# dangvansam/viet-asr

Hardware: AMD Instinct MI355X
Metric: real_time_factor (higher is better)
Workload: dtype f32 via 2xf16 split operands (22-bit significands, 3 f16 MFMA products per multiply, fp32 accumulate); 1 GPU; BASELINE configs[2]: quartznet15x5 greedy CTC, batch=64x10s 16kHz mono per GPU, wav in HBM -> collapsed ids; batch_per_gpu=64, parallelism=utterance-shard x1

## Files before the change

include/vasr_devtools.h:

```cpp
#ifndef VASR_DEVTOOLS_H_
#define VASR_DEVTOOLS_H_
#include "vasr.h"
#ifdef __cplusplus
extern "C" {
#endif

VASR_API int vasr_profile_bracket_overhead(vasr_stream stream, int n, double* out_us);
VASR_API int vasr_fused_tile_choice(int64_t tiles128, int compute_units);
VASR_API int vasr_fused_waves_choice(int kernel, int dual, int tile_cols);
VASR_API int vasr_bench_depthwise(const float* d_x, const float* d_w, const int32_t* d_lens, int batch, int channels,
                         int64_t frames, int kernel, float* d_y, vasr_stream stream);
VASR_API int vasr_bench_depthwise_layer(const float* d_x, const float* d_w, const int32_t* d_lens_in, const int32_t* d_lens_out,
                               int batch, int channels, int64_t frames_in, int kernel, int stride, int dilation, float* d_y,
                               uint32_t* d_amax, int amax_stride, vasr_stream stream);
VASR_API int vasr_depthwise_mfma_table_size(int kernel, int dilation);
VASR_API int vasr_pack_depthwise_taps(const float* h_w, int channels, int kernel, int dilation, uint32_t* h_table, float* h_inv);
VASR_API int vasr_bench_depthwise_mfma(const float* d_x, const uint32_t* d_taps, const float* d_tap_inv, const int32_t* d_lens,
                              int batch, int channels, int64_t frames, int kernel, int dilation, float* d_y,
                              uint32_t* d_amax, int amax_stride, vasr_stream stream);
VASR_API int vasr_pack_pointwise(const float* h_w, int cout, int cin, int m_pad, float* h_out);
VASR_API int vasr_conv_gemm_weights(const float* h_w, int cout, int cin, int kernel, float* h_out);
VASR_API int vasr_bench_pointwise(const float* d_x, const float* d_wt, const float* d_scale, const float* d_shift,
                         int batch, int cin, int cout, int64_t frames, float* d_y, vasr_stream stream);

VASR_API int vasr_bench_mfma_sustained(int gemm_mode, int workgroups, int steps, float* d_sink, double* flops, vasr_stream stream);

VASR_API int vasr_pack_pointwise_f16x2(const float* h_w, int cout, int cin, int m_pad, uint16_t* h_out, float* inv_scale);
VASR_API int vasr_bench_pointwise_f16x2(const float* d_x, const uint16_t* d_w16, float w_inv_scale, const float* d_scale,
                               const float* d_shift, int batch, int cin, int cout, int64_t frames, float* d_y,
                               uint32_t* d_amax, int amax_stride, vasr_stream stream);

VASR_API int vasr_pack_pointwise_bf16x3(const float* h_w, int cout, int cin, int m_pad, uint16_t* h_out);
VASR_API int vasr_bench_pointwise_bf16x3(const float* d_x, const uint16_t* d_w3, const float* d_scale, const float* d_shift,
                                int batch, int cin, int cout, int64_t frames, float* d_y, vasr_stream stream);

VASR_API int vasr_bench_groupnorm(const float* d_x, const int32_t* d_lens, int batch, int channels, int64_t frames,
                                  int norm_groups, int shuffle, const float* h_gamma, const float* h_beta, int relu, float* d_y,
                                  vasr_stream stream);
VASR_API int vasr_bench_ctc_head(const float* d_logits, int batch, int64_t frames, int num_classes, float* d_logp,
                                 int64_t* d_pred, vasr_stream stream);
#ifdef __cplusplus
}
#endif
#endif
```

viet-asr_amd/_lib.py:

```python
import ctypes as C
import os

import numpy as np
import torch

_HERE = os.path.dirname(os.path.abspath(__file__))
LIB_PATH = os.environ.get("VASR_LIB_PATH") or os.path.join(_HERE, "lib", "libvasr_hip.so")
DEV_LIB_PATH = os.environ.get("VASR_LIB_PATH") or os.path.join(_HERE, "lib", "libvasr_hip_dev.so")


class VasrError(RuntimeError):
    pass


class BlockDesc(C.Structure):
    _fields_ = [(n, C.c_int32) for n in
                ("filters", "repeat", "kernel", "stride", "dilation", "residual", "separable", "residual_dense")]


class FrontendDesc(C.Structure):
    _fields_ = [("sample_rate", C.c_int32), ("n_fft", C.c_int32), ("win_length", C.c_int32),
                ("hop_length", C.c_int32), ("n_mels", C.c_int32), ("preemph", C.c_float),
                ("log_guard", C.c_float), ("normalize", C.c_int32),
                ("h_window", C.POINTER(C.c_float)), ("h_filterbank", C.POINTER(C.c_float)),
# ... 66 lines not shown
    "vasr_beam_workgroups": (C.c_int, [C.c_int]),
    "vasr_beam_hash_init": (C.c_uint64, []),
    "vasr_beam_hash_step": (C.c_uint64, [C.c_uint64, C.c_uint64]),
    "vasr_last_error": (C.c_char_p, []),
    "vasr_version": (C.c_char_p, []),
    "vasr_abi_version": (C.c_int, []),
    "vasr_algorithmic_work": (C.c_int, [_P, C.c_int, C.c_int64, C.POINTER(C.c_double)]),
    "vasr_profile_begin": (C.c_int, [_P]),
    "vasr_profile_end": (C.c_int, [_P, C.POINTER(C.c_double), C.POINTER(C.c_int64), C.POINTER(C.c_double), C.POINTER(C.c_double)]),
    "vasr_padded_frames": (C.c_int64, [C.c_int64]),
}

DEV_SIGNATURES = {
    "vasr_pack_pointwise_f16x2": (C.c_int, [_P, C.c_int, C.c_int, C.c_int, _P, C.POINTER(C.c_float)]),
    "vasr_bench_pointwise_f16x2": (C.c_int, [_P, _P, C.c_float, _P, _P, C.c_int, C.c_int, C.c_int, C.c_int64, _P, _P,
                                             C.c_int, _P]),
    "vasr_depthwise_mfma_table_size": (C.c_int, [C.c_int, C.c_int]),
    "vasr_pack_depthwise_taps": (C.c_int, [_P, C.c_int, C.c_int, C.c_int, _P, _P]),
    "vasr_bench_depthwise_mfma": (C.c_int, [_P, _P, _P, _P, C.c_int, C.c_int, C.c_int64, C.c_int, C.c_int, _P, _P, C.c_int, _P]),
    "vasr_profile_bracket_overhead": (C.c_int, [_P, C.c_int, C.POINTER(C.c_double)]),
    "vasr_fused_tile_choice": (C.c_int, [C.c_int64, C.c_int]),
    "vasr_fused_waves_choice": (C.c_int, [C.c_int, C.c_int, C.c_int]),
    "vasr_pack_pointwise": (C.c_int, [_P, C.c_int, C.c_int, C.c_int, _P]),
    "vasr_conv_gemm_weights": (C.c_int, [_P, C.c_int, C.c_int, C.c_int, _P]),
    "vasr_pack_pointwise_bf16x3": (C.c_int, [_P, C.c_int, C.c_int, C.c_int, _P]),
    "vasr_bench_pointwise_bf16x3": (C.c_int, [_P, _P, _P, _P, C.c_int, C.c_int, C.c_int, C.c_int64, _P, _P]),
    "vasr_bench_mfma_sustained": (C.c_int, [C.c_int, C.c_int, C.c_int, _P, C.POINTER(C.c_double), _P]),
    "vasr_bench_depthwise": (C.c_int, [_P, _P, _P, C.c_int, C.c_int, C.c_int64, C.c_int, _P, _P]),
    "vasr_bench_depthwise_layer": (C.c_int, [_P, _P, _P, _P, C.c_int, C.c_int, C.c_int64, C.c_int, C.c_int, C.c_int, _P, _P,
                                             C.c_int, _P]),
    "vasr_bench_pointwise": (C.c_int, [_P, _P, _P, _P, C.c_int, C.c_int, C.c_int, C.c_int64, _P, _P]),
    "vasr_bench_groupnorm": (C.c_int, [_P, _P, C.c_int, C.c_int, C.c_int64, C.c_int, C.c_int, _P, _P, C.c_int, _P, _P]),
    "vasr_bench_ctc_head": (C.c_int, [_P, C.c_int, C.c_int64, C.c_int, _P, _P, _P]),
}

ABI_VERSION = 8

_lib = None
_dev = None


def _load(path, tables):
    if not os.path.exists(path):
        raise VasrError(
            f"{path} is missing: build it with `python -c 'import __graft_entry__ as g; g.build()'` "
            "(or `make -C viet-asr_amd/csrc`). There is no CPU fallback for this path.")
    l = C.CDLL(path)
    for table, required in tables:
        for name, (res, args) in table.items():
            fn = getattr(l, name, None)
            if fn is None:
                if required:
                    raise VasrError(f"{path} does not export {name}")
                continue
            fn.restype, fn.argtypes = res, args
    have = l.vasr_abi_version() if hasattr(l, "vasr_abi_version") else 0
    if have != ABI_VERSION:
        raise VasrError(f"{path} implements ABI {have}, these bindings expect {ABI_VERSION}: rebuild it (make -C viet-asr_amd/csrc)")
    return l


def lib():
    global _lib
    if _lib is None:
        _lib = _load(LIB_PATH, ((SIGNATURES, True), (DEV_SIGNATURES, False)))
    return _lib
# ... 147 lines not shown
```

viet-asr_amd/csrc/encoder_dw.hip:

```cpp
#include <cstdlib>

#include "vasr_internal.h"
#include "len_chain.h"
#include "vasr_device.h"

namespace vasr {

namespace {

constexpr int kTile = 512;

template <int K, int DIL = 1>
struct DwGeom {
  static constexpr int PAD = DIL > 1 ? (DIL * K) / 2 - 1 : K / 2;
  static constexpr int PADL = (PAD + 3) & ~3;
  static constexpr int OFF = PADL - PAD;
  static constexpr int NQ = (OFF + K + 3 + 3) / 4;
  static constexpr int WIN = 256 + 252 + 4 * NQ;
};

__device__ __forceinline__ void wave_sync() {
  __builtin_amdgcn_fence(__ATOMIC_RELEASE, "wavefront");
  __builtin_amdgcn_wave_barrier();
  __builtin_amdgcn_fence(__ATOMIC_ACQUIRE, "wavefront");
// ... 362 lines not shown
  const int t = t0 + threadIdx.x;
  int len_in = lens_in[b];
  if (len_in > frames_in) len_in = frames_in;
  const int64_t row = (int64_t)b * channels + c;
  const float* xr = x + row * ldx;
  const float* wc = w + (int64_t)c * K;
  const int span = 255 * stride + dil * (K - 1) + 1, s_base = t0 * stride - pad;
  const bool staged = span <= kSpan;
  if (staged) {
    for (int j = threadIdx.x; j < span; j += blockDim.x) {
      const int s = s_base + j;
      xs[j] = (s >= 0 && s < len_in) ? xr[s] : 0.f;
    }
    __syncthreads();
  }
  float acc = 0.f;
  if (t < ldy && t < lens_out[b]) {
    if (staged) {
      const float* xt = xs + threadIdx.x * stride;
      for (int k = 0; k < K; ++k) acc = fmaf(wc[k], xt[k * dil], acc);
    } else {
      const int s0 = t * stride - pad;
      for (int k = 0; k < K; ++k) {
        const int s = s0 + k * dil;
        if (s >= 0 && s < len_in) acc = fmaf(wc[k], xr[s], acc);
      }
    }
  }
  if (t < ldy) y[row * ldy + t] = acc;
  if (amax)
    amax_publish(amax, amax_stride, b, (c * gridDim.x + blockIdx.x) * 4 + (threadIdx.x >> 6), abs_bits(acc), threadIdx.x & 63);
}

__global__ void len_chain_kernel(const int64_t* __restrict__ seq, int batch, const LenStep* __restrict__ steps,
                                 int n_steps, int32_t* __restrict__ lens_tab, float* __restrict__ enc_len,
                                 const int64_t* __restrict__ wav_len, int hop, int frames_cap) {
  const int b = blockIdx.x * blockDim.x + threadIdx.x;
  len_chain_body(b, b < batch ? seq[b] : 0, batch, steps, n_steps, lens_tab, enc_len, wav_len, hop, frames_cap);
}

__global__ __launch_bounds__(256) void repad_kernel(const float* __restrict__ src, int64_t src_ld, int frames,
                                                    float* __restrict__ dst, int64_t dst_ld) {
  const int64_t r = blockIdx.y;
  for (int t = blockIdx.x * blockDim.x + threadIdx.x; t < dst_ld; t += gridDim.x * blockDim.x)
    dst[r * dst_ld + t] = t < frames ? src[r * src_ld + t] : 0.f;
}

template <int K>
void launch_dw_t(const float* x, int64_t ldx, const float* w, const int32_t* li, const int32_t* lo, int batch,
                 int channels, float* y, int64_t ldy, hipStream_t st, AmaxTab* amax) {
  const unsigned tiles = (unsigned)((ldy + kTile - 1) / kTile);
  unsigned* ap = amax ? amax->p : nullptr;
  const int as = amax ? amax->stride : 0;
  dim3 grid(channels / 4, batch, tiles);
  if (amax) amax->n = grid.x * 4 * tiles;
  VASR_LAUNCH((dw_conv_kernel<K, 1>), grid, dim3(256), 0, st, x, ldx, w, li, lo, channels, y, ldy, ap, as);
}

}

int depthwise_amax_slots(int channels, int64_t ldy) {
  return channels * (int)((ldy + 255) / 256) * 4;
}

static int launch_depthwise_impl(const float* x, int64_t ldx, int frames_in, const float* w, const int32_t* lens_in,
                                 const int32_t* lens_out, int batch, int channels, int kernel, int stride, int dilation,
// ... 15 lines not shown
  const bool pair = dev_switches().dw_pair;
  if (pair && aligned && stride == 1) {
    if (dilation == 2 && kernel == 87 && pad == 86)
      { launch_dw_pair<87, 2>(x, ldx, w, lens_in, lens_out, batch, channels, y, ldy, st, amax); return 0; }
    if (dilation == 1 && pad == kernel / 2) {
      switch (kernel) {
        case 33: { launch_dw_pair<33, 1>(x, ldx, w, lens_in, lens_out, batch, channels, y, ldy, st, amax); return 0; }
        case 39: { launch_dw_pair<39, 1>(x, ldx, w, lens_in, lens_out, batch, channels, y, ldy, st, amax); return 0; }
        case 51: { launch_dw_pair<51, 1>(x, ldx, w, lens_in, lens_out, batch, channels, y, ldy, st, amax); return 0; }
        case 63: { launch_dw_pair<63, 1>(x, ldx, w, lens_in, lens_out, batch, channels, y, ldy, st, amax); return 0; }
        case 75: { launch_dw_pair<75, 1>(x, ldx, w, lens_in, lens_out, batch, channels, y, ldy, st, amax); return 0; }
        default: break;
      }
    }
  }
  if (aligned && stride == 1 && dilation == 2 && kernel == 87 && pad == 86) {
    dim3 grid(channels / 4, batch, (unsigned)((ldy + kTile - 1) / kTile));
    if (amax) amax->n = grid.x * 4 * grid.z;
    VASR_LAUNCH((dw_conv_kernel<87, 1, 2>), grid, dim3(256), 0, st, x, ldx, w, lens_in, lens_out, channels,
                       y, ldy, amax ? amax->p : nullptr, amax ? amax->stride : 0);
    return 0;
  }
  const bool fast = aligned && stride == 1 && dilation == 1 && pad == kernel / 2;
  if (fast) {
    switch (kernel) {
      case 33: { launch_dw_t<33>(x, ldx, w, lens_in, lens_out, batch, channels, y, ldy, st, amax); return 0; }
      case 39: { launch_dw_t<39>(x, ldx, w, lens_in, lens_out, batch, channels, y, ldy, st, amax); return 0; }
      case 51: { launch_dw_t<51>(x, ldx, w, lens_in, lens_out, batch, channels, y, ldy, st, amax); return 0; }
      case 63: { launch_dw_t<63>(x, ldx, w, lens_in, lens_out, batch, channels, y, ldy, st, amax); return 0; }
      case 75: { launch_dw_t<75>(x, ldx, w, lens_in, lens_out, batch, channels, y, ldy, st, amax); return 0; }
      default: break;
    }
  }
  dim3 grid((unsigned)((ldy + 255) / 256), channels, batch);
  if (amax) amax->n = channels * grid.x * 4;
  VASR_LAUNCH(dw_conv_generic_kernel, grid, dim3(256), 0, st, x, ldx, frames_in, w, lens_in, lens_out,
                     channels, kernel, stride, dilation, pad, y, ldy, amax ? amax->p : nullptr, amax ? amax->stride : 0);
  return 0;
}

__global__ __launch_bounds__(256) void amax_kernel(const float* __restrict__ x, int64_t ld, int rows, int frames,
                                                   const int32_t* __restrict__ lens, unsigned* __restrict__ amax,
                                                   int amax_stride, int64_t bs) {
  const int b = blockIdx.y;
  int n = lens ? lens[b] : frames;
  n = n < frames ? n : frames;
  unsigned m = 0;
  for (int r = blockIdx.x; r < rows; r += gridDim.x) {
    const float* xr = x + (int64_t)b * bs + (int64_t)r * ld;
    for (int t = threadIdx.x; t < n; t += blockDim.x) m = max(m, abs_bits(xr[t]));
  }
  amax_publish(amax, amax_stride, b, blockIdx.x * 4 + (threadIdx.x >> 6), m, threadIdx.x & 63);
}

void launch_amax(const float* x, int64_t ld, int rows, int frames, const int32_t* lens, int batch, AmaxTab* amax,
                 hipStream_t st, int64_t batch_stride) {
  const int gx = rows < 64 ? rows : 64;
  amax->n = gx * 4;
  hipLaunchKernelGGL(amax_kernel, dim3(gx, batch), dim3(256), 0, st, x, ld, rows, frames, lens, amax->p, amax->stride,
                     batch_stride ? batch_stride : (int64_t)rows * ld);
}

void launch_len_chain(const int64_t* seq, int batch, const LenStep* d_steps, int n_steps, int32_t* lens_tab,
                      float* enc_len, hipStream_t st, const int64_t* wav_len, int hop, int frames_cap) {
  hipLaunchKernelGGL(len_chain_kernel, dim3((batch + 63) / 64), dim3(64), 0, st, seq, batch, d_steps, n_steps,
                     lens_tab, enc_len, wav_len, hop, frames_cap);
// ... 10 lines not shown
```

viet-asr_amd/csrc/vasr_api.cpp:

```cpp
#include <hip/hip_runtime.h>

#include <cmath>
#include <cstdarg>
#include <cstdio>
#include <cstdlib>
#include <cstring>
#include <map>
#include <memory>
#include <string>
#include <algorithm>
#include <vector>

#include "vasr.h"
#include "vasr_host.h"
#include "vasr_internal.h"

using namespace vasr;

namespace {
thread_local std::string g_err;
}

namespace vasr {

// ... 1053 lines not shown
      }
      int published;
      {
        ProfScope ps(h, kProfPointwise, st, 2.0 * W.cin * W.cout * (double)g_T * batch, 4.0 * W.m_pad * (double)dst_ld * batch);
        published = run_pointwise(h, a, W, st);
      }
      if (published < 0) return VASR_ERR_HIP;
      if (nrm) {
        if (run_norm(S.norm, dst, dst, (last_sub && B.has_res) ? R : nullptr, dst_ld, blk_ld, g_T, a.store_cols,
                     lens(S.pw.step + 1), enc_out ? nullptr : lens(S.pw.step + 1), act, published ? &a.amax_y : nullptr,
                     a.lens_y))
          return VASR_ERR_HIP;
      }
      if (S.se.d_w1) {
        if (run_se(S.se, dst, dst, dst_ld, g_T, a.store_cols, lens(S.pw.step + 1), enc_out ? nullptr : lens(S.pw.step + 1),
                   last_sub ? 1 : 0, 0, published ? &a.amax_y : nullptr, a.lens_y))
          return VASR_ERR_HIP;
      }
      cur = dst; cur_ld = dst_ld; cur_T = g_T;
      cur_amax = published ? a.amax_y : AmaxTab{};
    }
  }
  if (enc_amax) *enc_amax = cur_amax;
  return check_launch("encoder");
}

int run_decoder(vasr_handle* h, const float* encp, int64_t ld, int64_t T1, int batch, float* logits, float* logp,
                int64_t* pred, hipStream_t st, AmaxTab enc_amax = AmaxTab{}, const int32_t* own_frames = nullptr) {
  PwArgs a = pw_args(h, h->dec, encp, logits, ld, T1, batch);
  a.lens = own_frames;
  a.m_store = h->num_classes;
  ProfScope ps(h, kProfHead, st);
  a.amax_x = enc_amax;
  if (run_pointwise(h, a, h->dec, st) < 0) return VASR_ERR_HIP;
  launch_logsoftmax_argmax(logits, ld, (int64_t)h->num_classes * ld, batch, (int)T1, h->num_classes, logp, pred, st);
  return check_launch("decoder");
}

}

extern "C" {

const char* vasr_last_error(void) { return g_err.c_str(); }
const char* vasr_version(void) { return "vasr-hip 0.4 (gfx950)"; }
int vasr_abi_version(void) { return VASR_ABI_VERSION; }
int64_t vasr_padded_frames(int64_t frames) { return pad_frames(frames); }

int vasr_create(const vasr_model_desc* d, vasr_handle** out) {
  if (!d || !out) return fail(VASR_ERR_INVALID, "null argument");
  std::unique_ptr<vasr_handle> owner(new vasr_handle());
  vasr_handle* h = owner.get();
  if (d->frontend) {
    const vasr_frontend_desc& fe = *d->frontend;
    if (fe.n_fft != 512 || fe.n_mels != 64) {
      return fail(VASR_ERR_UNSUPPORTED, "front end supports n_fft=512, n_mels=64 (got %d, %d)", fe.n_fft, fe.n_mels);
    }
    if (fe.win_length <= 0 || fe.win_length > fe.n_fft || fe.hop_length <= 0 || fe.hop_length > 512 ||
        !fe.h_filterbank) {
      return fail(VASR_ERR_INVALID, "invalid window/hop/filterbank in front-end description");
    }
    h->has_frontend = true;
    h->fe = fe;
    h->fe_window.resize(fe.win_length);
    for (int i = 0; i < fe.win_length; ++i)
      h->fe_window[i] = fe.h_window ? fe.h_window[i]
                                    : (float)(0.5 - 0.5 * std::cos(2.0 * M_PI * i / (fe.win_length - 1)));
// ... 873 lines not shown
```

viet-asr_amd/csrc/vasr_devtools.cpp:

```cpp
#include <hip/hip_runtime.h>

#include <algorithm>
#include <cstdio>
#include <cstdlib>
#include <initializer_list>
#include <vector>

#include "vasr.h"
#include "vasr_devtools.h"
#include "vasr_host.h"
#include "vasr_internal.h"

using namespace vasr;

const vasr::DevSwitches& vasr::dev_switches() {
  static const DevSwitches sw = [] {
    DevSwitches s;
    auto num = [](const char* name, int dflt, std::initializer_list<int> allowed) {
      const char* e = getenv(name);
      if (!e) return dflt;
      const int v = atoi(e);
      for (int a : allowed) if (a == v) return v;
      fprintf(stderr, "vasr (devtools build): %s=%s is not a documented value -- refusing to guess\n", name, e);
      abort();
      return dflt;
    };
    s.pw3_tile = num("VASR_PW3_TILE", 0, {0, 1, 2, 3, 4, 5});
    s.pw_lat = num("VASR_PW_LAT", 1, {0, 1});
    s.dw_pair = num("VASR_DW_PAIR", 1, {0, 1}) != 0;
    s.dw_mfma = num("VASR_DW_MFMA", 1, {0, 1}) != 0;
    s.dw_upw = num("VASR_DW_UPW", 0, {0, 1, 2, 3, 4, 5, 6, 7, 8});
    s.fused = num("VASR_FUSED", 1, {0, 1}) != 0;
    s.fused_min_tiles = getenv("VASR_FUSED_MIN_TILES") ? atoi(getenv("VASR_FUSED_MIN_TILES")) : 0;
    s.fused_tile = num("VASR_FUSED_TILE", 0, {0, 64, 128});
    s.fused_waves = num("VASR_FUSED_WAVES", 0, {0, 8, 16});
    s.fused_residual = num("VASR_NO_FUSED_RESIDUAL", 0, {0, 1}) == 0;
    s.beam_group = num("VASR_BEAM_GROUP", -1, {-1, 0, 1, 4});
    s.no_grouped = num("VASR_NO_GROUPED", 0, {0, 1}) != 0;
    return s;
  }();
  return sw;
}

extern "C" {

int vasr_fused_tile_choice(int64_t tiles128, int compute_units) { return vasr::fused_tile_choice(tiles128, compute_units); }
int vasr_fused_waves_choice(int kernel, int dual, int tile_cols) {
  return vasr::fused_waves_choice(kernel, dual != 0, tile_cols, vasr::dev_switches().fused_waves);
}

static __global__ void dev_noop_kernel() {}

int vasr_profile_bracket_overhead(vasr_stream stream, int n, double* out_us) {
  if (n < 1 || n > 4096 || !out_us) return fail(VASR_ERR_INVALID, "bad argument");
  hipStream_t st = static_cast<hipStream_t>(stream);
  std::vector<hipEvent_t> ev(2 * (size_t)n);
  for (auto& e : ev) HIP_TRY(hipEventCreate(&e));
  for (int i = 0; i < n; ++i) {
    HIP_TRY(hipEventRecord(ev[2 * i], st));
    hipLaunchKernelGGL(dev_noop_kernel, dim3(1), dim3(64), 0, st);
    HIP_TRY(hipEventRecord(ev[2 * i + 1], st));
  }
  HIP_TRY(hipEventSynchronize(ev.back()));
  std::vector<float> t(n);
  for (int i = 0; i < n; ++i) HIP_TRY(hipEventElapsedTime(&t[i], ev[2 * i], ev[2 * i + 1]));
  for (auto& e : ev) (void)hipEventDestroy(e);
  std::sort(t.begin(), t.end());
  *out_us = 1e3 * (double)t[n / 2];
  return 0;
}

// ... 150 lines not shown
  const size_t nc = (size_t)channels, ws = (size_t)2 * batch * (channels + norm_groups);
  HIP_TRY(hipMalloc(&buf, (4 * nc + ws) * 4));
  float* f = reinterpret_cast<float*>(buf);
  int32_t* i32 = reinterpret_cast<int32_t*>(buf);
  NormLaunch a{};
  a.x = d_x; a.y = d_y; a.add = nullptr; a.ld = ld; a.ld_add = ld; a.bs = 0;
  a.channels = channels; a.groups = norm_groups; a.batch = batch; a.frames = (int)frames; a.store_cols = (int)ld;
  a.lens = d_lens; a.gamma = f; a.beta = f + nc; a.group_of = i32 + 2 * nc; a.members = i32 + 3 * nc;
  a.row_mean = f + 4 * nc; a.row_m2 = a.row_mean + (size_t)batch * channels;
  a.g_mean = a.row_m2 + (size_t)batch * channels; a.g_rstd = a.g_mean + (size_t)batch * norm_groups;
  a.zero_lens = d_lens; a.relu = relu;
  hipError_t e = hipMemcpyAsync(buf, t.gamma.data(), nc * 4, hipMemcpyHostToDevice, st);
  if (e == hipSuccess) e = hipMemcpyAsync(buf + nc * 4, t.beta.data(), nc * 4, hipMemcpyHostToDevice, st);
  if (e == hipSuccess) e = hipMemcpyAsync(buf + 2 * nc * 4, t.group_of.data(), nc * 4, hipMemcpyHostToDevice, st);
  if (e == hipSuccess) e = hipMemcpyAsync(buf + 3 * nc * 4, t.members.data(), nc * 4, hipMemcpyHostToDevice, st);
  if (e == hipSuccess) e = (hipError_t)launch_norm(a, st);
  if (e == hipSuccess) e = hipStreamSynchronize(st);
  (void)hipFree(buf);
  if (e != hipSuccess) return fail(VASR_ERR_HIP, "bench_groupnorm: %s", hipGetErrorString(e));
  return 0;
}

int vasr_bench_ctc_head(const float* d_logits, int batch, int64_t frames, int num_classes, float* d_logp, int64_t* d_pred,
                        vasr_stream stream) {
  if (!d_logits || batch < 1 || frames < 1 || frames > 0x7fffff00 || num_classes < 1 || num_classes > 128 || (!d_logp && !d_pred))
    return fail(VASR_ERR_INVALID, "bench_ctc_head: batch %d, frames %lld, num_classes %d (1..128), logp %s, pred %s", batch,
                (long long)frames, num_classes, d_logp ? "given" : "NULL", d_pred ? "given" : "NULL");
  const int64_t ld = pad_frames(frames);
  launch_logsoftmax_argmax(d_logits, ld, (int64_t)num_classes * ld, batch, (int)frames, num_classes, d_logp, d_pred,
                           static_cast<hipStream_t>(stream));
  return check_launch("bench_ctc_head");
}

}
```

viet-asr_amd/csrc/vasr_internal.h:

```cpp
#pragma once
#include <hip/hip_runtime.h>
#include <atomic>
#include <hip/hip_ext.h>
#include <stdint.h>
#include <stdlib.h>

namespace vasr {

struct DevSwitches {
  int pw3_tile = 0;
  int pw_lat = 1;
  bool dw_pair = true;
  bool dw_mfma = true;
  int dw_upw = 0;
  bool fused = true;
  int fused_min_tiles = 0;
  int fused_tile = 0;
  int fused_waves = 0;
  bool fused_residual = true;
  int beam_group = -1;
  bool no_grouped = false;
};
#ifdef VASR_DEVTOOLS
const DevSwitches& dev_switches();
#else
inline const DevSwitches& dev_switches() { static constexpr DevSwitches k{}; return k; }
#endif

struct LaunchProbe { hipEvent_t start = nullptr, stop = nullptr; };
extern thread_local LaunchProbe g_probe;
#define VASR_LAUNCH(kern, grid, block, lds, st, ...)                                                       \
  do {                                                                                                     \
    if (::vasr::g_probe.start) {                                                                           \
      hipExtLaunchKernelGGL(kern, grid, block, lds, st, ::vasr::g_probe.start, ::vasr::g_probe.stop, 0,   \
                            __VA_ARGS__);                                                                  \
      ::vasr::g_probe.start = nullptr;                                                                     \
    } else {                                                                                               \
      hipLaunchKernelGGL(kern, grid, block, lds, st, __VA_ARGS__);                                         \
    }                                                                                                      \
  } while (0)

inline hipError_t dyn_lds_opt_in(const void* kernel, int bytes, std::atomic<uint64_t>& done) {
  int dev = 0;
  if (hipGetDevice(&dev) != hipSuccess) dev = 0;
  const uint64_t bit = 1ull << (dev & 63);
  if (done.load(std::memory_order_relaxed) & bit) return hipSuccess;
  const hipError_t e = hipFuncSetAttribute(kernel, hipFuncAttributeMaxDynamicSharedMemorySize, bytes);
  if (e == hipSuccess) done.fetch_or(bit, std::memory_order_relaxed);
  return e;
}

#define VASR_LAUNCH_PART(first, last, kern, grid, block, lds, st, ...)                                     \
  do {                                                                                                     \
    if (::vasr::g_probe.start) {                                                                           \
// ... 153 lines not shown
int launch_se(const SeLaunch& a, hipStream_t st);

struct NormLaunch {
  const float* x; float* y; const float* add;
  int64_t ld, ld_add, bs;
  int channels, groups, batch, frames, store_cols;
  const int32_t* lens;
  const int32_t* group_of; const int32_t* members;
  const float* gamma; const float* beta;
  float* row_mean; float* row_m2;
  float* g_mean; float* g_rstd;
  const int32_t* zero_lens;
  int relu, act;
  AmaxTab* amax_y; const int32_t* lens_y;
};
bool norm_supported(int channels, int groups);
int launch_norm(const NormLaunch& a, hipStream_t st);

int launch_crop_or_pad(const float* in, int64_t ld_in, int batch, int feat, int frames, const int64_t* wav_len, int hop,
                       int audio_length, const int64_t* off, float* out, int64_t ld_out, int store_cols, int64_t* out_len,
                       hipStream_t st);
constexpr int kClassifyMaxChannels = 1024;
struct ClassifyLaunch {
  const float* x; int64_t ld;
  int batch, channels, frames, classes, pool_max, softmax;
  const float* w; const float* bias;
  float* pooled; float* out;
};
int launch_classifier(const ClassifyLaunch& a, hipStream_t st);

void launch_logsoftmax_argmax(const float* logits, int64_t row_ld, int64_t batch_stride, int batch, int frames,
                              int num_classes, float* logp, int64_t* pred, hipStream_t st);
void launch_argmax(const float* logp, int batch, int64_t frames, int num_classes, int64_t* pred, hipStream_t st);
void launch_ctc_collapse(const int64_t* pred, int batch, int64_t frames, int blank, int32_t* ids,
                         int32_t* id_len, hipStream_t st, const int64_t* wav_len = nullptr, int hop = 0,
                         const LenStep* steps = nullptr, int n_steps = 0);

constexpr int kMetricsMaxWidth = 4096;
constexpr int kMetricsMaxSpace = 8;
struct SpaceIds { int32_t id[kMetricsMaxSpace]; int n; };
int launch_error_counts(const int32_t* hyp, int hyp_width, const int32_t* hyp_len, const int32_t* ref, int ref_width,
                        const int32_t* ref_len, int batch, const SpaceIds& sp, int32_t* counts, hipStream_t st);
constexpr int kMetricsMaxScriptWidth = 1024;
int launch_error_ops(const int32_t* hyp, int hyp_width, const int32_t* hyp_len, const int32_t* ref, int ref_width,
                     const int32_t* ref_len, int batch, const SpaceIds& sp, int32_t* ops, int32_t* script, int32_t* script_len,
                     hipStream_t st);
constexpr int kMetricsMaxNbest = 65535;
int launch_nbest_error_counts(const int32_t* ids, int width, const int32_t* id_len, const int32_t* count, int nbest,
                              const int32_t* ref, int ref_width, const int32_t* ref_len, int batch, const SpaceIds& sp,
                              int32_t* slot_counts, int32_t* counts, int32_t* slot, hipStream_t st);

constexpr int kClassScoresMaxClasses = 65536;
constexpr int kClassScoresMaxK = 16;
int launch_class_scores(const float* logits, int batch, int classes, const int64_t* targets, int k, int32_t* topk_idx,
                        float* topk_val, float* topk_prob, int32_t* rank, float* loss, hipStream_t st);

constexpr int kCtcLossMaxWidth = 4096;
constexpr int kCtcLossLanes = 256;
constexpr int kCtcLossNarrowSlots = 4;
constexpr int kCtcLossWideSlots = 33;
int launch_ctc_loss(const float* logp, const int32_t* frames_in, int batch, int64_t frames, int classes, int blank,
                    const int32_t* tgt, int tgt_width, const int32_t* tgt_len, float* loss, hipStream_t st);

constexpr int kCtcAlignNarrowFrameBytes = 256;
constexpr int kCtcAlignWideFrameBytes = 2064;
constexpr int kCtcAlignNarrowBlock = 64;
// ... 47 lines not shown
```

Baseline: 130,200 audio-sec/wall-sec.

## Fuse CTC decoder GEMM with log-softmax/argmax and add stride-2 depthwise kernel

Adds a fused CTC head kernel that runs the f16x2-split decoder GEMM and computes log-softmax and argmax in the epilogue. This avoids writing logits to HBM and a separate softmax/argmax launch. It also adds a specialised stride-2 depthwise convolution kernel that stages a window in LDS and computes four outputs per lane. Both are on by default via switches, and the CTC head falls back to the old path when its constraints fail. The risk is extra code complexity and register/LDS pressure in the fused epilogue.

```diff
diff --git a/include/vasr_devtools.h b/include/vasr_devtools.h
--- a/include/vasr_devtools.h
+++ b/include/vasr_devtools.h
@@ -39,6 +39,10 @@
                                   vasr_stream stream);
 VASR_API int vasr_bench_ctc_head(const float* d_logits, int batch, int64_t frames, int num_classes, float* d_logp,
                                  int64_t* d_pred, vasr_stream stream);
+VASR_API int vasr_bench_ctc_head_f16x2(const float* d_x, const uint16_t* d_w16, float w_inv_scale, const float* d_scale,
+                                       const float* d_shift, const int32_t* d_own_frames, int batch, int cin, int num_classes,
+                                       int64_t frames, float* d_logits, float* d_logp, int64_t* d_pred, uint32_t* d_amax,
+                                       int amax_stride, vasr_stream stream);
 #ifdef __cplusplus
 }
 #endif
diff --git a/viet-asr_amd/_lib.py b/viet-asr_amd/_lib.py
--- a/viet-asr_amd/_lib.py
+++ b/viet-asr_amd/_lib.py
@@ -122,6 +122,8 @@
     "vasr_bench_pointwise": (C.c_int, [_P, _P, _P, _P, C.c_int, C.c_int, C.c_int, C.c_int64, _P, _P]),
     "vasr_bench_groupnorm": (C.c_int, [_P, _P, C.c_int, C.c_int, C.c_int64, C.c_int, C.c_int, _P, _P, C.c_int, _P, _P]),
     "vasr_bench_ctc_head": (C.c_int, [_P, C.c_int, C.c_int64, C.c_int, _P, _P, _P]),
+    "vasr_bench_ctc_head_f16x2": (C.c_int, [_P, _P, C.c_float, _P, _P, _P, C.c_int, C.c_int, C.c_int, C.c_int64, _P, _P, _P, _P,
+                                            C.c_int, _P]),
 }
 
 ABI_VERSION = 8
diff --git a/viet-asr_amd/csrc/ctc_head.hip b/viet-asr_amd/csrc/ctc_head.hip
--- /dev/null
+++ b/viet-asr_amd/csrc/ctc_head.hip
@@ -0,0 +1,318 @@
+#include <atomic>
+#include <type_traits>
+
+#include "vasr_internal.h"
+#include "vasr_device.h"
+
+namespace vasr {
+
+namespace {
+
+constexpr int BKC = 64;
+constexpr int STEPS = BKC / 16;
+
+template <int NW, int TN, int MT>
+struct HeadGeom {
+  static constexpr int WN = 32 * TN;
+  static constexpr int BN = WN * NW;
+  static constexpr int LR = WN / 4;
+  static constexpr int GP = 64 / LR;
+  static constexpr int NG = 8 / GP;
+  static constexpr int PPT = 4 * NG;
+  static constexpr int STAGE_BYTES = 2 * 2 * STEPS * 2 * WN * 16;
+  static constexpr int EPI_BYTES = 32 * 129 * 4;
+  static constexpr int WAVE_BYTES = STAGE_BYTES > EPI_BYTES ? STAGE_BYTES : EPI_BYTES;
+  static constexpr size_t LDS = (size_t)NW * WAVE_BYTES;
+};
+
+template <int NW, int TN, int MT, bool MASK>
+__global__ __launch_bounds__(64 * NW) void ctc_head_kernel(PwArgs a, float* __restrict__ logp, int64_t* __restrict__ pred,
+                                                           int tiles_t, int n_blocks) {
+  using G = HeadGeom<NW, TN, MT>;
+  constexpr int WN = G::WN, PPT = G::PPT;
+  extern __shared__ __attribute__((aligned(16))) uint4 smem[];
+  const int bid = xcd_remap(blockIdx.x, n_blocks);
+  const int b = bid / tiles_t;
+  const int lane = threadIdx.x & 63;
+  const int wave = __builtin_amdgcn_readfirstlane(threadIdx.x >> 6);
+  const int t0 = (bid % tiles_t) * G::BN + wave * WN;
+  if (t0 >= a.ldx) return;
+  if (!a.y && t0 >= a.frames) return;
+  uint4* Bs = smem + wave * (G::WAVE_BYTES / 16);
+  auto bs = [&](int buf, int plane, int s, int kb, int n) -> uint4& {
+    return Bs[(((buf * 2 + plane) * STEPS + s) * 2 + kb) * WN + n];
+  };
+  const int kh = lane >> 5, l31 = lane & 31;
+  const int len = MASK ? a.lens[b] : 0;
+  float xs = 1.f, out_scale = 1.f;
+  const float* __restrict__ xb = a.x + (int64_t)b * a.K * a.ldx + t0;
+  const int ksteps = a.K / 16;
+  const uint4* __restrict__ ap = reinterpret_cast<const uint4*>(a.wt) + lane;
+  const int64_t a_tile = (int64_t)ksteps * 2 * 64;
+
+  f32x16 acc[MT][TN];
+#pragma unroll
+  for (int i = 0; i < MT; ++i)
+#pragma unroll
+    for (int j = 0; j < TN; ++j)
+#pragma unroll
+      for (int r = 0; r < 16; ++r) acc[i][j][r] = 0.f;
+
+  const int c4 = lane % G::LR, gb = lane / G::LR;
+  constexpr int SSETS = 2;
+  float rr[SSETS][PPT][8];
+  auto gload = [&](int k0, auto set_tag) {
+    auto& r = rr[decltype(set_tag)::value % SSETS];
+    k0 = k0 < a.K - BKC ? k0 : a.K - BKC;
+    const float* __restrict__ base = xb + (int64_t)k0 * a.ldx + 4 * c4;
+#pragma unroll
+    for (int q = 0; q < G::NG; ++q) {
+      const float* __restrict__ src = base + (int64_t)(8 * (gb + G::GP * q)) * a.ldx;
+#pragma unroll
+      for (int e = 0; e < 8; ++e) {
+        const v4f v = *reinterpret_cast<const v4f*>(src + (int64_t)e * a.ldx);
+        r[4 * q][e] = v.x; r[4 * q + 1][e] = v.y; r[4 * q + 2][e] = v.z; r[4 * q + 3][e] = v.w;
+      }
+    }
+  };
+  auto sstore_half = [&](int buf, auto set_tag, int p, int h) {
+    const auto& r = rr[decltype(set_tag)::value % SSETS];
+    const int n = 4 * c4 + (p & 3), g = gb + G::GP * (p >> 2);
+    const bool keep = !MASK || (t0 + n < len);
+    float x[4];
+#pragma unroll
+    for (int e = 0; e < 4; ++e) x[e] = keep ? r[p][4 * h + e] : 0.f;
+    unsigned hh[2], ll[2];
+#pragma unroll
+    for (int q = 0; q < 2; ++q) {
+      const v2f v = {x[2 * q] * xs, x[2 * q + 1] * xs};
+      const f16x2 hv = __builtin_convertvector(v, f16x2);
+      const v2f rs = v - __builtin_convertvector(hv, v2f);
+      hh[q] = __builtin_bit_cast(unsigned, hv);
+      ll[q] = __builtin_bit_cast(unsigned, __builtin_convertvector(rs, f16x2));
+    }
+    reinterpret_cast<uint2*>(&bs(buf, 0, g >> 1, g & 1, n))[h] = make_uint2(hh[0], hh[1]);
+    reinterpret_cast<uint2*>(&bs(buf, 1, g >> 1, g & 1, n))[h] = make_uint2(ll[0], ll[1]);
+  };
+
+  uint4 aw[2][MT][2];
+  uint4 (&af)[MT][2] = aw[0];
+  uint4 (&an)[MT][2] = aw[1];
+  auto aload = [&](int s, uint4 (&dst)[MT][2]) {
+    const int sc = s < ksteps ? s : ksteps - 1;
+#pragma unroll
+    for (int i = 0; i < MT; ++i)
+#pragma unroll
+      for (int p = 0; p < 2; ++p) dst[i][p] = ap[i * a_tile + ((int64_t)sc * 2 + p) * 64];
+  };
+
+  using S0 = std::integral_constant<int, 0>;
+  using S1 = std::integral_constant<int, 1>;
+  const int nchunks = a.K / BKC;
+  {
+    unsigned amv[8];
+    amax_request(a.amax_x.p, a.amax_x.stride, a.amax_x.n, b, lane, amv);
+    gload(0, S0{});
+    aload(0, af);
+    const unsigned mx = amax_collect(a.amax_x.p, a.amax_x.stride, a.amax_x.n, b, lane, amv);
+    float inv;
+    f16_scale(mx, &xs, &inv);
+    out_scale = inv * a.w_inv_scale;
+#pragma unroll
+    for (int p = 0; p < PPT; ++p) {
+      sstore_half(0, S0{}, p, 0);
+      sstore_half(0, S0{}, p, 1);
+    }
+    gload(BKC, S0{});
+  }
+  wave_fence();
+
+  auto run_chunk = [&](const int c, auto cur, auto nxt, auto last_tag) {
+    constexpr bool LAST = decltype(last_tag)::value;
+    constexpr int HALVES = 2 * PPT;
+    const int cn = c + 1;
+    uint4 bf[2][2];
+#pragma unroll
+    for (int p = 0; p < 2; ++p) bf[0][p] = bs(c & 1, p, 0, kh, l31);
+#pragma unroll
+    for (int s = 0; s < STEPS; ++s) {
+      aload(c * STEPS + s + 1, an);
+      if (!LAST && s == 0) gload((c + SSETS) * BKC, nxt);
+      __builtin_amdgcn_sched_barrier(0);
+      uint4 (&cw)[MT][2] = af;
+#pragma unroll
+      for (int j = 0; j < TN; ++j) {
+        const int g = s * TN + j;
+        const int cur_f = g & 1, nxt_f = cur_f ^ 1;
+        if (j + 1 < TN) {
+#pragma unroll
+          for (int p = 0; p < 2; ++p) bf[nxt_f][p] = bs(c & 1, p, s, kh, (j + 1) * 32 + l31);
+        } else if (s + 1 < STEPS) {
+#pragma unroll
+          for (int p = 0; p < 2; ++p) bf[nxt_f][p] = bs(c & 1, p, s + 1, kh, l31);
+        }
+#pragma unroll
+        for (int i = 0; i < MT; ++i)
+          acc[i][j] = __builtin_amdgcn_mfma_f32_32x32x16_f16(__builtin_bit_cast(f16x8, cw[i][1]), __builtin_bit_cast(f16x8, bf[cur_f][0]), acc[i][j], 0, 0, 0);
+#pragma unroll
+        for (int i = 0; i < MT; ++i)
+          acc[i][j] = __builtin_amdgcn_mfma_f32_32x32x16_f16(__builtin_bit_cast(f16x8, cw[i][0]), __builtin_bit_cast(f16x8, bf[cur_f][1]), acc[i][j], 0, 0, 0);
+#pragma unroll
+        for (int i = 0; i < MT; ++i)
+          acc[i][j] = __builtin_amdgcn_mfma_f32_32x32x16_f16(__builtin_bit_cast(f16x8, cw[i][0]), __builtin_bit_cast(f16x8, bf[cur_f][0]), acc[i][j], 0, 0, 0);
+        if (!LAST && j == 0) {
+          const int h0 = s * HALVES / STEPS, h1 = (s + 1) * HALVES / STEPS;
+#pragma unroll
+          for (int hv = h0; hv < h1; ++hv) sstore_half(cn & 1, cur, hv >> 1, hv & 1);
+        }
+      }
+#pragma unroll
+      for (int i = 0; i < MT; ++i)
+#pragma unroll
+        for (int p = 0; p < 2; ++p) af[i][p] = an[i][p];
+    }
+    wave_fence();
+  };
+  {
+    int c = 0;
+    for (; c + 2 < nchunks; c += 2) {
+      run_chunk(c, S0{}, S1{}, std::false_type{});
+      run_chunk(c + 1, S1{}, S0{}, std::false_type{});
+    }
+    run_chunk(c, S0{}, S1{}, std::false_type{});
+    run_chunk(c + 1, S1{}, S0{}, std::true_type{});
+  }
+
+  const int V = a.m_store;
+  v4f scv[MT][4], shv[MT][4];
+#pragma unroll
+  for (int i = 0; i < MT; ++i)
+#pragma unroll
+    for (int q = 0; q < 4; ++q) {
+      scv[i][q] = *reinterpret_cast<const v4f*>(a.scale + i * 32 + 8 * q + 4 * kh);
+      shv[i][q] = *reinterpret_cast<const v4f*>(a.shift + i * 32 + 8 * q + 4 * kh);
+    }
+  float* tile = reinterpret_cast<float*>(Bs);
+  const int VP = V | 1;
+#pragma unroll
+  for (int j = 0; j < TN; ++j) {
+    const int tj = t0 + 32 * j, t = tj + l31;
+    float x[MT][16];
+    float mx = -INFINITY;
+#pragma unroll
+    for (int i = 0; i < MT; ++i)
+#pragma unroll
+      for (int q = 0; q < 4; ++q)
+#pragma unroll
+        for (int r = 0; r < 4; ++r) {
+          const int m = i * 32 + 8 * q + 4 * kh + r;
+          float v = acc[i][j][4 * q + r];
+          v *= out_scale;
+          v = fmaf(v, scv[i][q][r], shv[i][q][r]);
+          x[i][4 * q + r] = v;
+          if (m < V) {
+            mx = fmaxf(mx, v);
+            if (a.y) a.y[((int64_t)b * V + m) * a.ldy + t] = v;
+          }
+        }
+    if (tj >= a.frames) continue;
+    mx = fmaxf(mx, __shfl_xor(mx, 32));
+    float s = 0.f;
+#pragma unroll
+    for (int i = 0; i < MT; ++i)
+#pragma unroll
+      for (int q = 0; q < 4; ++q) {
+        float e4[4], p4[4];
+#pragma unroll
+        for (int r = 0; r < 4; ++r) e4[r] = expf(x[i][4 * q + r] - mx);
+#pragma unroll
+        for (int r = 0; r < 4; ++r) p4[r] = __shfl_xor(e4[r], 32);
+#pragma unroll
+        for (int r = 0; r < 4; ++r) {
+          const float v = kh ? p4[r] : e4[r];
+          s = i * 32 + 8 * q + r < V ? s + v : s;
+        }
+#pragma unroll
+        for (int r = 0; r < 4; ++r) {
+          const float v = kh ? e4[r] : p4[r];
+          s = i * 32 + 8 * q + 4 + r < V ? s + v : s;
+        }
+      }
+    const float ls = logf(s);
+    float best = -INFINITY;
+    int arg = 0;
+#pragma unroll
+    for (int i = 0; i < MT; ++i)
+#pragma unroll
+      for (int q = 0; q < 4; ++q)
+#pragma unroll
+        for (int r = 0; r < 4; ++r) {
+          const int m = i * 32 + 8 * q + 4 * kh + r;
+          if (m < V) {
+            const float lp = (x[i][4 * q + r] - mx) - ls;
+            if (lp > best) { best = lp; arg = m; }
+            if (logp) tile[l31 * VP + m] = lp;
+          }
+        }
+    {
+      const float ob = __shfl_xor(best, 32);
+      const int oa = __shfl_xor(arg, 32);
+      if (ob > best || (ob == best && oa < arg)) arg = oa;
+    }
+    if (pred && kh == 0 && t < a.frames) pred[(int64_t)b * a.frames + t] = arg;
+    if (logp) {
+      wave_fence();
+      const int n = min(32, a.frames - tj) * V;
+      float* out = logp + ((int64_t)b * a.frames + tj) * V;
+      for (int i = lane; i < n; i += 64) {
+        const int r = i / V;
+        out[i] = tile[r * VP + (i - r * V)];
+      }
+      wave_fence();
+    }
+  }
+}
+
+template <int NW, int TN, int MT, bool MASK>
+int launch_h(const PwArgs& a, float* logp, int64_t* pred, hipStream_t st) {
+  using G = HeadGeom<NW, TN, MT>;
+  const int tiles_t = (int)((a.ldx + G::BN - 1) / G::BN);
+  const int n_blocks = tiles_t * a.batch;
+  auto kern = ctc_head_kernel<NW, TN, MT, MASK>;
+  static std::atomic<uint64_t> lds_opted{0};
+  const hipError_t attr = dyn_lds_opt_in(reinterpret_cast<const void*>(kern), (int)G::LDS, lds_opted);
+  if (attr != hipSuccess) return (int)attr;
+  VASR_LAUNCH(kern, dim3(n_blocks), dim3(64 * NW), G::LDS, st, a, logp, pred, tiles_t, n_blocks);
+  return 0;
+}
+
+template <int NW, int TN, bool MT4 = true>
+int launch_f(const PwArgs& a, float* logp, int64_t* pred, hipStream_t st) {
+  const int mt = (a.m_store + 31) / 32;
+  const bool mask = a.lens != nullptr;
+  switch (mt) {
+    case 1: return mask ? launch_h<NW, TN, 1, true>(a, logp, pred, st) : launch_h<NW, TN, 1, false>(a, logp, pred, st);
+    case 2: return mask ? launch_h<NW, TN, 2, true>(a, logp, pred, st) : launch_h<NW, TN, 2, false>(a, logp, pred, st);
+    case 3: return mask ? launch_h<NW, TN, 3, true>(a, logp, pred, st) : launch_h<NW, TN, 3, false>(a, logp, pred, st);
+    default:
+      if constexpr (MT4) return mask ? launch_h<NW, TN, 4, true>(a, logp, pred, st) : launch_h<NW, TN, 4, false>(a, logp, pred, st);
+      else return launch_f<4, 1>(a, logp, pred, st);
+  }
+}
+
+}
+
+int launch_ctc_head(const PwArgs& a, float* logp, int64_t* pred, int form, hipStream_t st) {
+  const int V = a.m_store;
+  if (V < 1 || V > 128 || (V + 31) / 32 * 32 > a.M || a.K < 2 * BKC || a.K % (2 * BKC) || a.ldx % kTimeTile || a.frames < 1 ||
+      a.frames > a.ldx || !a.amax_x.p || a.x2 || a.res || a.conv_cin || a.bsx || a.groups > 1 || a.zero_from || a.amax_y.p ||
+      (reinterpret_cast<uintptr_t>(a.x) & 15) || (a.y && a.ldy < a.ldx) || (!a.y && !logp && !pred))
+    return -1;
+  switch (form) {
+    case 4: return launch_f<4, 2>(a, logp, pred, st);
+    case 8: return launch_f<8, 1, false>(a, logp, pred, st);
+    default: return launch_f<4, 1>(a, logp, pred, st);
+  }
+}
+
+}
diff --git a/viet-asr_amd/csrc/encoder_dw.hip b/viet-asr_amd/csrc/encoder_dw.hip
--- a/viet-asr_amd/csrc/encoder_dw.hip
+++ b/viet-asr_amd/csrc/encoder_dw.hip
@@ -418,6 +418,96 @@
     amax_publish(amax, amax_stride, b, (c * gridDim.x + blockIdx.x) * 4 + (threadIdx.x >> 6), abs_bits(acc), threadIdx.x & 63);
 }
 
+template <int K>
+struct Stride2Geom {
+  static constexpr int PAD = K / 2;
+  static constexpr int PADL = (PAD + 3) & ~3;
+  static constexpr int OFF = PADL - PAD;
+  static constexpr int NW = OFF + K + 6;
+  static constexpr int NQ = (NW + 3) / 4;
+  static constexpr int NLD = (2 * 63 + NQ + 63) / 64;
+  static constexpr int WIN4 = NLD * 64;
+};
+
+template <int K>
+__global__ __launch_bounds__(256) void dw_stride2_kernel(const float* __restrict__ x, int64_t ldx, int frames_in,
+                                                         const float* __restrict__ w,
+                                                         const int32_t* __restrict__ lens_in,
+                                                         const int32_t* __restrict__ lens_out, int channels,
+                                                         float* __restrict__ y, int64_t ldy, unsigned* __restrict__ amax,
+                                                         int amax_stride) {
+  using G = Stride2Geom<K>;
+  __shared__ v4f lds4[4 * G::WIN4];
+  const int lane = threadIdx.x & 63;
+  const int wave = __builtin_amdgcn_readfirstlane(threadIdx.x >> 6);
+  const int c = blockIdx.x * 4 + wave, b = blockIdx.y, tile = blockIdx.z;
+  const int t0 = tile * 256;
+  int len_in = lens_in[b];
+  if (len_in > frames_in) len_in = frames_in;
+  const int len_out = lens_out[b];
+  const int64_t row = (int64_t)b * channels + c;
+  const float* xr = x + row * ldx;
+  v4f* win4 = lds4 + wave * G::WIN4;
+
+  const int s0 = 2 * t0 - G::PADL;
+  v4f stage[G::NLD];
+#pragma unroll
+  for (int j = 0; j < G::NLD; ++j) {
+    const int s = s0 + 4 * (lane + 64 * j);
+    int sc = s < 0 ? 0 : s;
+    sc = sc > (int)ldx - 4 ? (int)ldx - 4 : sc;
+    stage[j] = *reinterpret_cast<const v4f*>(xr + sc);
+  }
+  const float* wg = w + (int64_t)c * K;
+  float wc[K];
+#pragma unroll
+  for (int k = 0; k < K; ++k) wc[k] = wg[k];
+#pragma unroll
+  for (int k = 0; k < K; ++k) asm volatile("" : "+s"(wc[k]));
+#pragma unroll
+  for (int j = 0; j < G::NLD; ++j) {
+    const int s = s0 + 4 * (lane + 64 * j);
+    const int n = s < 0 ? 0 : len_in - s;
+    v4f v = stage[j];
+    v.x = n > 0 ? v.x : 0.f;
+    v.y = n > 1 ? v.y : 0.f;
+    v.z = n > 2 ? v.z : 0.f;
+    v.w = n > 3 ? v.w : 0.f;
+    win4[lane + 64 * j] = v;
+  }
+  wave_sync();
+  float xw[4 * G::NQ];
+#pragma unroll
+  for (int q = 0; q < G::NQ; ++q) {
+    const v4f v = win4[2 * lane + q];
+    xw[4 * q] = v.x; xw[4 * q + 1] = v.y; xw[4 * q + 2] = v.z; xw[4 * q + 3] = v.w;
+  }
+  float acc[4] = {0.f, 0.f, 0.f, 0.f};
+#pragma unroll
+  for (int k = 0; k < K; ++k)
+#pragma unroll
+    for (int r = 0; r < 4; ++r) acc[r] = fmaf(wc[k], xw[G::OFF + 2 * r + k], acc[r]);
+  const int t = t0 + 4 * lane;
+  v4f o;
+#pragma unroll
+  for (int r = 0; r < 4; ++r) o[r] = t + r < len_out ? acc[r] : 0.f;
+  unsigned m = 0;
+  if (t < ldy) {
+    *reinterpret_cast<v4f*>(y + row * ldy + t) = o;
+    m = max(max(abs_bits(o.x), abs_bits(o.y)), max(abs_bits(o.z), abs_bits(o.w)));
+  }
+  if (amax) amax_publish(amax, amax_stride, b, c * gridDim.z + tile, m, lane);
+}
+
+template <int K>
+void launch_dw_stride2(const float* x, int64_t ldx, int frames_in, const float* w, const int32_t* li, const int32_t* lo,
+                       int batch, int channels, float* y, int64_t ldy, hipStream_t st, AmaxTab* amax) {
+  dim3 grid(channels / 4, batch, (unsigned)((ldy + 255) / 256));
+  if (amax) amax->n = channels * grid.z;
+  VASR_LAUNCH((dw_stride2_kernel<K>), grid, dim3(256), 0, st, x, ldx, frames_in, w, li, lo, channels, y, ldy,
+              amax ? amax->p : nullptr, amax ? amax->stride : 0);
+}
+
 __global__ void len_chain_kernel(const int64_t* __restrict__ seq, int batch, const LenStep* __restrict__ steps,
                                  int n_steps, int32_t* __restrict__ lens_tab, float* __restrict__ enc_len,
                                  const int64_t* __restrict__ wav_len, int hop, int frames_cap) {
@@ -499,6 +589,19 @@
       default: break;
     }
   }
+  if (dev_switches().dw_stride2 && aligned && stride == 2 && dilation == 1 && kernel % 2 == 1 && kernel <= 33 &&
+      pad == kernel / 2 && ldx % kTimeTile == 0 && ldy % kTimeTile == 0 && ldx <= (1 << 30) && ldy <= (1 << 30) &&
+      frames_in <= ldx) {
+    switch (kernel) {
+#define VASR_DW_S2(KK) \
+      case KK: { launch_dw_stride2<KK>(x, ldx, frames_in, w, lens_in, lens_out, batch, channels, y, ldy, st, amax); return 0; }
+      VASR_DW_S2(1) VASR_DW_S2(3) VASR_DW_S2(5) VASR_DW_S2(7) VASR_DW_S2(9) VASR_DW_S2(11) VASR_DW_S2(13) VASR_DW_S2(15)
+      VASR_DW_S2(17) VASR_DW_S2(19) VASR_DW_S2(21) VASR_DW_S2(23) VASR_DW_S2(25) VASR_DW_S2(27) VASR_DW_S2(29) VASR_DW_S2(31)
+      VASR_DW_S2(33)
+#undef VASR_DW_S2
+      default: break;
+    }
+  }
   dim3 grid((unsigned)((ldy + 255) / 256), channels, batch);
   if (amax) amax->n = channels * grid.x * 4;
   VASR_LAUNCH(dw_conv_generic_kernel, grid, dim3(256), 0, st, x, ldx, frames_in, w, lens_in, lens_out,
diff --git a/viet-asr_amd/csrc/vasr_api.cpp b/viet-asr_amd/csrc/vasr_api.cpp
--- a/viet-asr_amd/csrc/vasr_api.cpp
+++ b/viet-asr_amd/csrc/vasr_api.cpp
@@ -1109,6 +1109,15 @@
   a.m_store = h->num_classes;
   ProfScope ps(h, kProfHead, st);
   a.amax_x = enc_amax;
+  if (h->sw.ctc_head && h->gemm_mode == 3 && h->dec.d_w16 && enc_amax.p && (logp || pred)) {
+    PwArgs f = a;
+    f.wt = reinterpret_cast<const float*>(h->dec.d_w16);
+    f.w_inv_scale = h->dec.w16_inv;
+    f.y = nullptr;
+    const int e = launch_ctc_head(f, logp, pred, h->sw.ctc_head, st);
+    if (e > 0) return fail(VASR_ERR_HIP, "ctc head: %s", hipGetErrorString((hipError_t)e));
+    if (e == 0) return check_launch("decoder");
+  }
   if (run_pointwise(h, a, h->dec, st) < 0) return VASR_ERR_HIP;
   launch_logsoftmax_argmax(logits, ld, (int64_t)h->num_classes * ld, batch, (int)T1, h->num_classes, logp, pred, st);
   return check_launch("decoder");
diff --git a/viet-asr_amd/csrc/vasr_devtools.cpp b/viet-asr_amd/csrc/vasr_devtools.cpp
--- a/viet-asr_amd/csrc/vasr_devtools.cpp
+++ b/viet-asr_amd/csrc/vasr_devtools.cpp
@@ -29,7 +29,8 @@
     s.pw_lat = num("VASR_PW_LAT", 1, {0, 1});
     s.dw_pair = num("VASR_DW_PAIR", 1, {0, 1}) != 0;
     s.dw_mfma = num("VASR_DW_MFMA", 1, {0, 1}) != 0;
-    s.dw_upw = num("VASR_DW_UPW", 0, {0, 1, 2, 3, 4, 5, 6, 7, 8});
+    s.dw_stride2 = num("VASR_DW_STRIDE2", 1, {0, 1}) != 0;
+    s.dw_upw =num("VASR_DW_UPW", 0, {0, 1, 2, 3, 4, 5, 6, 7, 8});
     s.fused = num("VASR_FUSED", 1, {0, 1}) != 0;
     s.fused_min_tiles = getenv("VASR_FUSED_MIN_TILES") ? atoi(getenv("VASR_FUSED_MIN_TILES")) : 0;
     s.fused_tile = num("VASR_FUSED_TILE", 0, {0, 64, 128});
@@ -37,6 +38,7 @@
     s.fused_residual = num("VASR_NO_FUSED_RESIDUAL", 0, {0, 1}) == 0;
     s.beam_group = num("VASR_BEAM_GROUP", -1, {-1, 0, 1, 4});
     s.no_grouped = num("VASR_NO_GROUPED", 0, {0, 1}) != 0;
+    s.ctc_head = num("VASR_CTC_HEAD", 1, {0, 1, 2, 4, 8});
     return s;
   }();
   return sw;
@@ -253,4 +255,32 @@
   return check_launch("bench_ctc_head");
 }
 
-}
+int vasr_bench_ctc_head_f16x2(const float* d_x, const uint16_t* d_w16, float w_inv_scale, const float* d_scale,
+                              const float* d_shift, const int32_t* d_own_frames, int batch, int cin, int num_classes,
+                              int64_t frames, float* d_logits, float* d_logp, int64_t* d_pred, uint32_t* d_amax, int amax_stride,
+                              vasr_stream stream) {
+  if (!d_x || !d_w16 || !d_scale || !d_shift || !d_amax || amax_stride < 256 || batch < 1 || frames < 1 || frames > 0x7fffff00 ||
+      num_classes < 1 || num_classes > 128 || !pointwise_split_supported(128, cin, 0) || (!d_logits && !d_logp && !d_pred))
+    return fail(VASR_ERR_INVALID, "bench_ctc_head_f16x2: bad argument");
+  const int64_t ld = pad_frames(frames);
+  hipStream_t st = static_cast<hipStream_t>(stream);
+  AmaxTab ax{d_amax, amax_stride, 0};
+  launch_amax(d_x, ld, cin, (int)frames, nullptr, batch, &ax, st);
+  PwArgs a = pw_args(d_w16, d_scale, d_shift, 128, cin, d_x, d_logits, ld, frames, batch);
+  a.lens = d_own_frames;
+  a.m_store = num_classes;
+  a.amax_x = ax; a.w_inv_scale = w_inv_scale;
+  const int form = dev_switches().ctc_head;
+  int e = form ? launch_ctc_head(a, d_logp, d_pred, form, st) : -1;
+  if (e > 0) return fail(VASR_ERR_HIP, "ctc head: %s", hipGetErrorString((hipError_t)e));
+  if (e < 0) {
+    if (!d_logits) return fail(VASR_ERR_INVALID, "bench_ctc_head_f16x2: the three-launch path needs d_logits");
+    e = launch_pointwise_split(a, 2, st);
+    if (e) return fail(VASR_ERR_HIP, "pointwise GEMM: %s", hipGetErrorString((hipError_t)e));
+    if (d_logp || d_pred)
+      launch_logsoftmax_argmax(d_logits, ld, (int64_t)num_classes * ld, batch, (int)frames, num_classes, d_logp, d_pred, st);
+  }
+  return check_launch("bench_ctc_head_f16x2");
+}
+
+}
diff --git a/viet-asr_amd/csrc/vasr_internal.h b/viet-asr_amd/csrc/vasr_internal.h
--- a/viet-asr_amd/csrc/vasr_internal.h
+++ b/viet-asr_amd/csrc/vasr_internal.h
@@ -12,6 +12,7 @@
   int pw_lat = 1;
   bool dw_pair = true;
   bool dw_mfma = true;
+  bool dw_stride2 = true;
   int dw_upw = 0;
   bool fused = true;
   int fused_min_tiles = 0;
@@ -20,6 +21,7 @@
   bool fused_residual = true;
   int beam_group = -1;
   bool no_grouped = false;
+  int ctc_head = 1;
 };
 #ifdef VASR_DEVTOOLS
 const DevSwitches& dev_switches();
@@ -239,6 +241,7 @@
 void launch_logsoftmax_argmax(const float* logits, int64_t row_ld, int64_t batch_stride, int batch, int frames,
                               int num_classes, float* logp, int64_t* pred, hipStream_t st);
 void launch_argmax(const float* logp, int batch, int64_t frames, int num_classes, int64_t* pred, hipStream_t st);
+int launch_ctc_head(const PwArgs& a, float* logp, int64_t* pred, int form, hipStream_t st);
 void launch_ctc_collapse(const int64_t* pred, int batch, int64_t frames, int blank, int32_t* ids,
                          int32_t* id_len, hipStream_t st, const int64_t* wav_len = nullptr, int hop = 0,
                          const LenStep* steps = nullptr, int n_steps = 0);
```

New measurement: 130,800 audio-sec/wall-sec, median of 6. About the same (+0.4%).
